# zjuzly/MultiViewStitch

Hardware: AMD Instinct MI355X
Metric: nonrigid_outer_iterations_per_sec (higher is better)
Workload: dtype f64

## Files before the change

multiviewstitch_amd/csrc/deform_handle.cpp:

```cpp
#include "deform_host.h"
#include <chrono>

int check_params(const mvs_deform_params* p) {
    if (!p) { mvs_set_error("params is NULL"); return MVS_E_INVALID_ARG; }
    if (p->top_k < 1 || p->top_k > 8 || p->graph_k < 0 || p->graph_k > 63 || p->smooth_sweeps < 0 ||
        p->arap_iters < 1 || p->arap_iters > 8 || p->cg_max_iters < 1 || !(p->cg_tol > 0)) {
        mvs_set_error("params out of range (top_k 1..8, graph_k 0..63, arap_iters 1..8, cg_tol > 0)");
        return MVS_E_INVALID_ARG;
    }
    return MVS_OK;
}

static void free_nodes(mvs_deform_s* h) {
    if (h->arena_nodes) { (void)hipFree(h->arena_nodes); h->arena_nodes = nullptr; }
    h->d_nodes = nullptr; h->d_nbr = nullptr; h->d_node_pts = nullptr; h->d_node_nrm = nullptr; h->d_ctrl_raw = nullptr;
    h->d_ctrl_a = nullptr; h->d_ctrl_b = nullptr; h->d_valid = nullptr; h->d_d2min = nullptr; h->d_counts = nullptr;
    h->d_records = nullptr; h->d_top_idx = nullptr; h->d_heavy = nullptr; h->d_heavy2 = nullptr;
    h->d_prev_d2 = nullptr; h->d_prev_node = nullptr; h->d_knn_ws = nullptr;
    h->d_near_prev = nullptr; h->d_lim = nullptr; h->d_mid = nullptr; h->d_mid2 = nullptr; h->d_ng_sync = nullptr;
    h->near_age = 0; h->graph_prev_nn = 0;
    h->prev_valid = false;
    h->d_ctrl_final = nullptr; h->K = 0; h->nbr_k = 0; h->h_nodes.clear();
    h->graph_ready_nn = 0; h->weights_ready = false; h->heavy_pending = nullptr;
}
// ... 58 lines not shown
    if (!h) return MVS_OK;
    (void)hipSetDevice(h->device);
    if (h->stream) (void)hipStreamSynchronize(h->stream);
    free_nodes(h);
    for (void* a : {h->arena_mesh, h->arena_tab, h->arena_target, h->arena_probe}) if (a) (void)hipFree(a);
    if (h->d_slots) (void)hipFree(h->d_slots);
    if (h->d_cheb) (void)hipFree(h->d_cheb);
    if (h->d_sh) { (void)hipFree(h->d_sh); h->d_sh = nullptr; }
    if (h->h_ctl) { (void)hipHostFree((void*)h->h_ctl); h->h_ctl = nullptr; }
    if (h->timing.h_sample) { (void)hipHostFree(h->timing.h_sample); h->timing.h_sample = nullptr; }
    for (auto& pr : h->timing.pending) { (void)hipEventDestroy(pr.second.first); (void)hipEventDestroy(pr.second.second); }
    for (hipEvent_t e : h->timing.event_pool) (void)hipEventDestroy(e);
    if (h->own_stream) stream_release(h->device, h->own_stream);
    delete h;
    return MVS_OK;
}

static int install_nodes(mvs_deform_s* h, const int32_t* vertex_idx, int64_t K) {
    free_nodes(h);
    h->K = K;
    h->h_nodes.assign(vertex_idx, vertex_idx + K);
    const size_t ws_bytes = K >= 1024 ? knn_grid_ws_bytes((int)K) : 0;
    auto lay = [&](Arena& a) {
        h->d_heavy = a.take<int32_t>((size_t)K + 1); h->d_heavy2 = a.take<int32_t>((size_t)K + 1);
        h->d_valid = a.take<uint8_t>((size_t)K);
        h->d_nodes = a.take<int32_t>(K); h->d_node_pts = a.take<double>((size_t)K * 3); h->d_node_nrm = a.take<double>((size_t)K * 3);
        h->d_ctrl_raw = a.take<double>((size_t)K * 3); h->d_ctrl_a = a.take<double>((size_t)K * 3); h->d_ctrl_b = a.take<double>((size_t)K * 3);
        h->d_d2min = a.take<float>(K); h->d_counts = a.take<int32_t>((size_t)K * 2);
        h->d_prev_d2 = a.take<float>(K); h->d_prev_node = a.take<double>((size_t)K * 3);
        h->d_near_prev = a.take<double>((size_t)K * 3); h->d_lim = a.take<float>(K);
        h->d_mid = a.take<int32_t>((size_t)K + 1); h->d_mid2 = a.take<int32_t>((size_t)K + 1);
        h->d_ng_sync = a.take<unsigned long long>(32);
        h->d_records = a.take<mvs_cand>((size_t)K * 8); h->d_top_idx = a.take<int64_t>((size_t)K * 8);
        h->d_nbr = a.take<int32_t>((size_t)K * 64);
        h->d_knn_ws = ws_bytes ? (void*)a.take<char>(ws_bytes) : nullptr;
    };
    {
        Arena a; lay(a);
        HIPCHK(hipMalloc(&h->arena_nodes, a.off + 256));
        Arena b; b.base = (char*)h->arena_nodes; lay(b);
    }
    HIPCHK(hipMemsetAsync(h->d_heavy, 0, sizeof(int32_t), h->stream)); HIPCHK(hipMemsetAsync(h->d_heavy2, 0, sizeof(int32_t), h->stream));
    HIPCHK(hipMemsetAsync(h->d_mid, 0, sizeof(int32_t), h->stream)); HIPCHK(hipMemsetAsync(h->d_mid2, 0, sizeof(int32_t), h->stream));
    HIPCHK(hipMemsetAsync(h->d_ng_sync, 0, sizeof(unsigned long long) * 32, h->stream));
    h->ng_pass = 0;
    HIPCHK(hipMemsetAsync(h->d_valid, 0, (size_t)std::max<int64_t>(K, 1), h->stream));
    h->heavy_flip = 0;
    HIPCHK(hipMemsetAsync(h->d_is_ctrl, 0, sizeof(int32_t) * h->V, h->stream));
    if (K) HIPCHK(hipMemcpyAsync(h->d_nodes, h->h_nodes.data(), sizeof(int32_t) * K, hipMemcpyHostToDevice, h->stream));
    launch_gather_nodes(h->d_pts, h->d_nrm, h->d_nodes, (int)K, h->d_node_pts, h->d_node_nrm, h->stream, h->d_is_ctrl);
    if (K) HIPCHK(hipMemcpyAsync(h->d_ctrl_raw, h->d_node_pts, sizeof(double) * K * 3, hipMemcpyDeviceToDevice, h->stream));
    h->d_ctrl_final = h->d_ctrl_raw;
    h->cg_iters = 0;
    for (int i = 0; i < 8; ++i) { h->cg_plan[i] = 0; h->ras_plan[i] = 0; h->bump_seq[i] = 0; h->ras_hist_n[i] = 0; }
    h->ras_mix_any = 0; h->ras_mix_calm = 0; h->assoc_passes = 0;
    HIPCHK(hipMemsetAsync(h->d_ctl, 0, sizeof(double) * 4, h->stream));
    h->ras_a = 0.0; h->ras_m = 0;
    return MVS_OK;
}

int mvs_deform_set_nodes(mvs_deform_t h, const int32_t* vertex_idx, int64_t K) {
    MVS_TRACE();
    if (!h || K < 0 || (K > 0 && !vertex_idx)) { mvs_set_error("bad arguments"); return MVS_E_INVALID_ARG; }
    HIPCHK(hipSetDevice(h->device));
    std::vector<char> seen(h->V, 0);
    for (int64_t k = 0; k < K; ++k) {
        const int v = vertex_idx[k];
        if (v < 0 || v >= h->V) { mvs_set_error("node %lld: vertex index out of range", (long long)k); return MVS_E_INVALID_ARG; }
        if (seen[v]) { mvs_set_error("node %lld: vertex %d listed twice", (long long)k, v); return MVS_E_INVALID_ARG; }
        seen[v] = 1;
    }
    return install_nodes(h, vertex_idx, K);
}

int mvs_deform_set_vertices(mvs_deform_t h, const double* points, const double* normals) {
    MVS_TRACE();
    if (!h || !points) { mvs_set_error("bad arguments"); return MVS_E_INVALID_ARG; }
    HIPCHK(hipSetDevice(h->device));
    HIPCHK(hipStreamSynchronize(h->stream));
    HIPCHK(hipMemcpyAsync(h->d_pts, points, sizeof(double) * 3 * (size_t)h->V, hipMemcpyHostToDevice, h->stream));
    if (normals) HIPCHK(hipMemcpyAsync(h->d_nrm, normals, sizeof(double) * 3 * (size_t)h->V, hipMemcpyHostToDevice, h->stream));
    if (h->K > 0) {
        launch_gather_nodes(h->d_pts, h->d_nrm, h->d_nodes, (int)h->K, h->d_node_pts, h->d_node_nrm, h->stream);
        HIPCHK(hipMemcpyAsync(h->d_ctrl_raw, h->d_node_pts, sizeof(double) * h->K * 3, hipMemcpyDeviceToDevice, h->stream));
        HIPCHK(hipMemsetAsync(h->d_valid, 0, (size_t)h->K, h->stream));
        h->d_ctrl_final = h->d_ctrl_raw;
    }
    h->graph_ready_nn = 0; h->weights_ready = false; h->heavy_pending = nullptr; h->graph_in_local = false;
    h->near_age = 0;
    HIPCHK(hipStreamSynchronize(h->stream));
    return mvs_check_hip(hipGetLastError(), "set_vertices");
}

int mvs_deform_sample_nodes(mvs_deform_t h, int knn, int64_t* K) {
    MVS_TRACE();
    if (!h || knn < 1 || knn > 64) { mvs_set_error("knn must be 1..64"); return MVS_E_INVALID_ARG; }
    HIPCHK(hipSetDevice(h->device));
    const int64_t V = h->V;
    const auto t0 = std::chrono::steady_clock::now();
    auto lap = [&](const char* what) {
        if (mvs_debug_level()) fprintf(stderr, "[mvs] sample_nodes: %s at %.3f ms\n", what, std::chrono::duration<double, std::milli>(std::chrono::steady_clock::now() - t0).count());
    };
    const size_t tab_bytes = (sizeof(int32_t) * (size_t)V * knn + 255) & ~(size_t)255;
    const size_t ws_bytes = V >= 1024 ? knn_grid_ws_bytes((int)V) : 0;
    int32_t* tab = nullptr;
    int rc;
    {
// ... 146 lines not shown
```

multiviewstitch_amd/csrc/deform_iterate.cpp:

```cpp
#include "deform_host.h"

extern "C" {

int mvs_deform_iterate(mvs_deform_t h, const mvs_deform_params* p, int n_outer, mvs_deform_stats* stats) {
    MVS_TRACE();
    int rc = ready(h, p, true);
    if (rc) return rc;
    if (n_outer < 0) return MVS_E_INVALID_ARG;
    int done = 0;
    if (!stats && h->cg_iters > 0) {
        const CgPlan cg = probe_cg(h, *p);
        for (int o = 0; o < n_outer; ++o) {
            enqueue_assoc_local(h, *p);
            rc = enqueue_solve(h, *p, h->d_ctrl_raw, true, cg, true);
            if (rc) return rc;
        }
        return MVS_OK;
    }
    int status = MVS_OK;
    BatchAcc acc;
    acc.st = h->last;
    while (done < n_outer) {
        const bool calibrated = h->cg_iters > 0;
        const int batch = calibrated ? std::min(n_outer - done, MAX_BATCH) : 1;
        CgPlan cg = probe_cg(h, *p);
        for (int o = 0; o < batch; ++o) {
            if (calibrated && o > 0) {
                if ((rc = throttle(h))) return rc;
                peek_ring(h, *p, use_ras(h, *p));
                cg = probe_cg(h, *p);
            }
            enqueue_assoc_local(h, *p);
            rc = enqueue_solve(h, *p, h->d_ctrl_raw, true, cg);
            if (rc) return rc;
        }
        mvs_deform_stats st;
        rc = harvest(h, *p, cg, &st);
        if (rc < 0) return rc;
        if (rc > 0) status = rc;
        acc.add(st);
        done += batch;
    }
    acc.finish(&h->last, done);
    if (stats) *stats = h->last;
    return status;
}

int mvs_deform_assoc_dmin(mvs_deform_t h, const mvs_deform_params* p, float* d2min_dev) {
    MVS_TRACE();
    int rc = ready(h, p, true);
    if (rc) return rc;
    if (!d2min_dev) return MVS_E_INVALID_ARG;
    h->near_age = 0;
    Tic t = tic(h, "assoc");
    launch_assoc_dmin(h->grid, h->d_node_pts, (int)h->K, d2min_dev, h->stream, h->prev_valid ? h->d_prev_d2 : nullptr, h->d_prev_node);
    toc(t, 1);
    return mvs_check_hip(hipGetLastError(), "assoc_dmin");
}
int mvs_deform_assoc_select(mvs_deform_t h, const mvs_deform_params* p, const float* d2min_dev, mvs_cand* records_dev,
                            int32_t* counts_dev) {
    MVS_TRACE();
    int rc = ready(h, p, true);
    if (rc) return rc;
    if (!d2min_dev || !records_dev || !counts_dev) return MVS_E_INVALID_ARG;
// ... 112 lines not shown
```

multiviewstitch_amd/csrc/deform_pass.cpp:

```cpp
#include "deform_host.h"

AssocLists assoc_lists(const mvs_deform_s* h, int flip) {
    if (flip) return {h->d_heavy2, h->d_heavy, h->d_mid2, h->d_mid};
    return {h->d_heavy, h->d_heavy2, h->d_mid, h->d_mid2};
}

void enqueue_assoc_local(mvs_deform_s* h, const mvs_deform_params& p) {
    Tic t = tic(h, "assoc");
    const int K = (int)h->K;
    const AssocLists l = assoc_lists(h, h->heavy_flip);
    int32_t *cur = l.heavy, *nxt = l.heavy_next, *mcur = l.mid, *mnxt = l.mid_next;
    h->heavy_flip ^= 1;
    if (h->near_age >= 2 && h->grid.P > 0 && K > 0 && p.graph_k + 1 <= 16 && MVS_KNOB("MVS_ASSOC_BOUNDED", 1, 0, 1) != 0.0) {
        const int nn = p.graph_k + 1;
        const bool graph_here = h->d_knn_ws != nullptr && knn_grid_is_single(K) && ensure_nbr(h, nn) == MVS_OK;
        const bool bounded_graph = graph_here && h->graph_prev_nn == nn && K >= nn;
        const bool w = graph_here && use_ras(h, p);
        const bool build_in_all = graph_here && assoc_all_builds_grid(K) && MVS_KNOB("MVS_NG_IN_ALL", 1, 0, 1) != 0.0;
        launch_assoc_prep(h->grid, h->d_node_pts, K, h->d_d2min, h->d_near_prev, h->d_lim, cur, mcur, (graph_here && !build_in_all) ? h->d_knn_ws : nullptr, h->stream);
        launch_assoc_all(h->grid, h->d_node_pts, h->d_node_nrm, K, p, h->d_lim, h->d_d2min, h->d_records, h->d_counts, cur, mcur, nxt, mnxt, h->d_ctrl_raw,
                         h->d_valid, h->d_top_idx, nn, h->d_nbr, graph_here ? h->d_knn_ws : nullptr, bounded_graph, w ? &h->sell : nullptr, h->d_pts,
                         arap_grid_blocks(h->sell), h->stream, build_in_all ? h->d_ng_sync : nullptr, build_in_all ? ++h->ng_pass : 0);
        h->assoc_passes++;
        h->near_age++;
// ... 162 lines not shown

void finalize_pass(mvs_deform_s* h, const mvs_deform_params& p, const RasPlan& rp, const RasPass& c, const SolveState& st) {
    hipStream_t s = h->stream;
    const int K = (int)h->K, V = (int)h->V;
    double* host_ctl = const_cast<double*>(h->h_ctl);
    Tic t = tic(h, "finalize");
    int n = 1;
    if (p.update_normals) {
        launch_arap_finalize(h->sell, p.arap_iters, p.arap_tol, h->d_energy, st.x_cur, h->d_pts, h->d_info, nullptr, nullptr, nullptr, p.cg_tol, h->d_ctl, c.slot, host_ctl, st.prev_scal, s, c.nl, c.demand_local, (double)(h->seq_enqueued + 1));
        launch_vertex_normals(h->d_pts, h->d_faces, h->d_vf_ptr, h->d_vf, V, h->d_nrm, s);
        launch_gather_nodes(h->d_pts, h->d_nrm, h->d_nodes, K, h->d_node_pts, h->d_node_nrm, s);
        n = 3;
    } else {
        launch_arap_finalize(h->sell, p.arap_iters, p.arap_tol, h->d_energy, st.x_cur, h->d_pts, h->d_info, h->d_nrm, h->d_node_pts, h->d_node_nrm, p.cg_tol, h->d_ctl, c.slot, host_ctl, st.prev_scal, s, c.nl, c.demand_local, (double)(h->seq_enqueued + 1));
    }
    toc(t, n);
    if (st.sampling) {
        auto& T = h->timing;
        const int ss = ras_slot_size(h);
        const size_t nslots = (size_t)rp.total(p.arap_iters);
        T.sample_off.push_back(T.sample_used);
        (void)hipMemcpy2DAsync(T.h_sample + T.sample_used, 8 * sizeof(double), h->d_ras_slots + 3 * (size_t)h->ras.NPpad, (size_t)ss * sizeof(double),
                               8 * sizeof(double), nslots, hipMemcpyDeviceToHost, s);
        T.sample_used += nslots * 8;
    }
}

}

int enqueue_solve(mvs_deform_s* h, const mvs_deform_params& p, const double* ctrl_src, bool graph_smooth, const CgPlan& plan, bool safe_local) {
    Smoothed sm;
    sm.ctrl = ctrl_src;
    if (graph_smooth) {
        int rc = graph_and_smooth(h, p, &sm);
        if (rc) return rc;
    }
    if (!sm.last_sweep.out) h->d_ctrl_final = const_cast<double*>(sm.ctrl);
    const bool ras = use_ras(h, p);
    if (ras) update_mix_state(h, p.arap_iters);
    const RasPlan rp = probe_ras(h);
    int rc = ras ? ensure_ras_slots(h, p.arap_iters) : ensure_slots(h, p.arap_iters, plan);
    if (rc) return rc;
    weights_and_prepare(h, sm, ras);
    RasPass c;
    c.slot = (int)(h->seq_enqueued % MVS_RING);
    c.fused = ras && ras_can_fuse_local(h);
    c.safe_local = safe_local || h->saw_abandon;
    c.nl = ras ? ras_local_parts(h) : 0;
    c.demand_local = (c.fused && !c.safe_local) ? 1 : 0;
    SolveState st;
    st.x_cur = h->d_sol;
    st.sampling = ras && h->timing.mode == 3 && timed(h, "cg") && sample_room(h, rp.total(p.arap_iters));
    if (st.sampling) h->timing.sample_pass_first.push_back((int)h->timing.samples.size());
    if (ras) ras_solves(h, p, rp, c, st);
    else cg_solves(h, p, plan, c.slot);
    finalize_pass(h, p, rp, c, st);
    h->graph_ready_nn = 0; h->weights_ready = false;
    h->seq_enqueued++;
    return MVS_OK;
}
```

multiviewstitch_amd/csrc/deform_plan.cpp:

```cpp
#include "deform_host.h"
#include <sched.h>

constexpr int RAS_SPARES = 1;
static int ras_spares(int used) { return RAS_SPARES + used / 8; }
#define RAS_A_FLOOR MVS_KNOB("MVS_RAS_FLOOR", 0.01, 0.001, 0.06)
constexpr double PEEK_AT = 1.0;

constexpr int RAS_FIRST_PLANS[8] = {7, 6, 5, 5, 5, 5, 5, 5};
constexpr int RAS_MAX_SWEEPS = 128;
#define RAS_MIX_PLAN ((int)MVS_KNOB("MVS_MIX_PLAN", 11, 2, 128))
constexpr int RAS_MIX_OFF = 7, RAS_MIX_CALM = 16;
void update_mix_state(mvs_deform_s* h, int arap_iters) {
    bool any_long = false, all_short = true;
    for (int it = 0; it < arap_iters; ++it) {
        if (h->ras_plan[it] >= RAS_MIX_PLAN) any_long = true;
        if (h->ras_plan[it] > RAS_MIX_OFF) all_short = false;
    }
    if (any_long) { h->ras_mix_any = 1; h->ras_mix_calm = 0; }
    else if (h->ras_mix_any) {
        if (!all_short) h->ras_mix_calm = 0;
        else if (++h->ras_mix_calm >= RAS_MIX_CALM) { h->ras_mix_any = 0; h->ras_mix_calm = 0; }
    }
}

RasPlan probe_ras(const mvs_deform_s* h) {
    RasPlan r;
    for (int i = 0; i < 8; ++i) r.n[i] = h->ras_plan[i] > 0 ? h->ras_plan[i] : RAS_FIRST_PLANS[i];
    if (h->ras_mix_any) for (int i = 0; i < 8; ++i) r.n[i] = std::max(r.n[i], RAS_MIX_PLAN);
    const int cap = h->dbg.plan_cap > 0 ? h->dbg.plan_cap : (int)MVS_KNOB("MVS_RAS_PLAN_CAP", 0, 0, 128);
    if (cap > 0) for (int i = 0; i < 8; ++i) r.n[i] = std::min(r.n[i], cap);
    return r;
}

int ensure_ras_slots(mvs_deform_s* h, int arap_iters) {
    if ((int64_t)RAS_MAX_SWEEPS * arap_iters > h->ras_slots_cap || !h->d_ras_slots) { mvs_set_error("sweep slots not provisioned"); return MVS_E_STATE; }
    return MVS_OK;
}

int ensure_slots(mvs_deform_s* h, int arap_iters, const CgPlan& cg) {
    int64_t need = cg.total_slots(arap_iters) * MVS_CG_SLOT;
    if (need > h->slots_cap) {
        need += need / 2;
        if (h->d_slots) (void)hipFree(h->d_slots);
        int rc = dmalloc(&h->d_slots, (size_t)need);
        if (rc) return rc;
        h->slots_cap = need;
    }
    return MVS_OK;
}

constexpr int THROTTLE_LAG = 3;

int throttle(mvs_deform_s* h) {
    if (!h->h_ctl) return MVS_OK;
    for (unsigned spins = 0;; ++spins) {
        const uint64_t done = (uint64_t)h->h_ctl[MVS_CTL_SEQ];
        if (h->seq_enqueued <= done + THROTTLE_LAG) return MVS_OK;
        if ((spins & 0x3ff) == 0x3ff) {
            const hipError_t e = hipStreamQuery(h->stream);
            if (e == hipSuccess) return MVS_OK;
            if (e != hipErrorNotReady) return mvs_check_hip(e, "stream (throttle)");
            sched_yield();
        }
    }
}

void peek_ring(mvs_deform_s* h, const mvs_deform_params& p, bool ras) {
    if (!h->h_ctl) return;
    uint64_t done = (uint64_t)h->h_ctl[MVS_CTL_SEQ];
    const uint64_t due = h->seq_enqueued > (uint64_t)THROTTLE_LAG ? h->seq_enqueued - THROTTLE_LAG : 0;
    if (done > due) done = due;
    uint64_t q = h->seq_peeked;
    if (q >= done) return;
    if (done > MVS_RING && q < done - MVS_RING) q = done - MVS_RING;
    const double tol2 = PEEK_AT * PEEK_AT * p.cg_tol * p.cg_tol;
    const bool plan_lowering = MVS_KNOB("MVS_PLAN_LOWER", 1, 0, 1) != 0.0;
    for (; q < done; ++q) {
        const volatile double* row = h->h_ctl + MVS_CTL_RING + (q % MVS_RING) * 8;
        const volatile double* used = h->h_ctl + MVS_CTL_USED + (q % MVS_RING) * 8;
        for (int it = 0; it < p.arap_iters; ++it) {
            const double rel2 = row[it];
            if (rel2 < 0.0) continue;
            int want = 0;
            if (ras) {
                if (h->ras_plan[it] <= 0) continue;
                const int u = (int)used[it];
                if (u != 0) {
                    const int ran = std::abs(u) + (u < 0 ? 1 : 0);
                    want = ran + ras_spares(ran);
                    int* hist = h->ras_hist[it];
                    if (h->ras_hist_n[it] == 4) { hist[0] = hist[1]; hist[1] = hist[2]; hist[2] = hist[3]; hist[3] = ran; }
                    else hist[h->ras_hist_n[it]++] = ran;
                    const int HN = (int)MVS_KNOB("MVS_PLAN_HIST", 4, 1, 4);
                    if (plan_lowering && h->ras_hist_n[it] >= HN && u > 0) {
                        int m = 0;
                        for (int k = h->ras_hist_n[it] - HN; k < h->ras_hist_n[it]; ++k) m = std::max(m, hist[k]);
                        const int low = m + ras_spares(m);
                        if (low < h->ras_plan[it] && want <= low) {
                            if (mvs_debug_level()) fprintf(stderr, "[mvs] pass %llu solve %d: plan %d -> %d (the last four passes ran <= %d sweeps)\n",
                                                                (unsigned long long)q, it, h->ras_plan[it], low, m);
                            h->ras_plan[it] = low;
                        }
                    }
                }
                if (rel2 > tol2) want = std::max(want, h->ras_plan[it] + ras_spares(h->ras_plan[it]) + 1);
                want = std::min(RAS_MAX_SWEEPS, want);
                if (want > h->ras_plan[it]) {
                    if (mvs_debug_level()) fprintf(stderr, "[mvs] pass %llu solve %d ran %d of %d sweeps (ended at %.2e of cg_tol): plan %d from pass %llu on\n",
                                                        (unsigned long long)q, it, std::abs(u), h->ras_plan[it], std::sqrt(rel2) / p.cg_tol, want, (unsigned long long)h->seq_enqueued);
                    h->ras_plan[it] = want;
                }
            } else if (h->cg_plan[it] > 0 && rel2 > tol2 && q >= h->bump_seq[it]) {
                h->cg_plan[it] = std::min(p.cg_max_iters, h->cg_plan[it] + std::max(2, h->cg_plan[it] / 8));
                h->bump_seq[it] = h->seq_enqueued;
            }
        }
    }
    h->seq_peeked = done;
}

namespace {
struct Judgement {
    double worst2 = 0.0, last_worst2 = 0.0; int solves = 0, missed = 0; bool esc = false; double last_row[8];
    int rows = 0; int used[MVS_RING][8];
};
int read_judgement(mvs_deform_s* h, const mvs_deform_params& p, Judgement* j) {
    double ctl[MVS_CTL_SIZE];
    HIPCHK(hipMemcpyAsync(ctl, h->d_ctl, sizeof ctl, hipMemcpyDeviceToHost, h->stream));
    HIPCHK(hipStreamSynchronize(h->stream));
    j->esc = ctl[MVS_CTL_ESC] != 0.0;
    for (int it = 0; it < 8; ++it)
        if (ctl[MVS_CTL_GAVEUP + it] > h->gaveup_seen[it]) {
            h->gaveup_seen[it] = ctl[MVS_CTL_GAVEUP + it];
            h->saw_abandon = true;
        }
    if (mvs_debug_level()) fprintf(stderr, "[mvs] predicted stops: true / predicted residual (running maximum) %.2f\n", std::sqrt(std::max(1.0, ctl[MVS_CTL_PSAFE])));
    j->worst2 = ctl[MVS_CTL_WORST];
    j->missed = (int)ctl[MVS_CTL_MISSED];
    j->solves = (int)ctl[MVS_CTL_SOLVES];
    const double* row = ctl + MVS_CTL_RING + ((h->seq_enqueued + MVS_RING - 1) % MVS_RING) * 8;
    for (int it = 0; it < 8; ++it) { j->last_row[it] = row[it]; if (it < p.arap_iters && row[it] > j->last_worst2) j->last_worst2 = row[it]; }
    {
        const uint64_t since = std::min<uint64_t>(h->seq_enqueued - h->seq_harvested, MVS_RING);
        j->rows = (int)since;
        for (uint64_t q = 0; q < since; ++q) {
            const double* u = ctl + MVS_CTL_USED + ((h->seq_enqueued - 1 - q) % MVS_RING) * 8;
            for (int it = 0; it < 8; ++it) { const int v = (int)u[it]; j->used[q][it] = v < 0 ? 1 - v : v; }
        }
        h->seq_harvested = h->seq_enqueued;
    }
    HIPCHK(hipMemsetAsync(h->d_ctl, 0, sizeof(double) * 4, h->stream));
    h->seq_peeked = h->seq_enqueued;
    return MVS_OK;
}
int judged_status(const Judgement& j, const mvs_deform_params& p) {
    if (j.missed == 0) return MVS_OK;
    mvs_set_error("%d of %d global solves ended above cg_tol = %.1e (worst relative residual %.3e)%s", j.missed, j.solves, p.cg_tol,
                  std::sqrt(j.worst2), j.esc ? "; the device switched the remaining solves to the strong local-solve coefficients" : "");
    return MVS_W_UNCONVERGED;
}

struct PassReadback {
    std::vector<double> ered;
    int32_t info[8];
    std::vector<uint8_t> valid;
    Judgement jd;
    explicit PassReadback(const mvs_deform_s* h) : ered(MVS_ERED_SIZE), valid(h->K) {}
    int run() const { return info[0]; }
    int download(mvs_deform_s* h, const mvs_deform_params& p) {
        HIPCHK(hipMemcpyAsync(ered.data(), h->d_energy, sizeof(double) * MVS_ERED_SIZE, hipMemcpyDeviceToHost, h->stream));
        HIPCHK(hipMemcpyAsync(info, h->d_info, sizeof info, hipMemcpyDeviceToHost, h->stream));
        if (h->K) HIPCHK(hipMemcpyAsync(valid.data(), h->d_valid, (size_t)h->K, hipMemcpyDeviceToHost, h->stream));
        return read_judgement(h, p, &jd);
    }
    mvs_deform_stats fill(mvs_deform_s* h, const mvs_deform_params& p, int cg_iters, int launches, int active, mvs_deform_stats* st) const {
        mvs_deform_stats out{};
        out.arap_iters_run = run();
        out.cg_iters = cg_iters;
        for (int i = 0; i < 8; ++i) out.energy[i] = i < p.arap_iters ? ered[MVS_ERED_FIN + i] : 0.0;
        out.cg_rel_residual = std::sqrt(std::max(0.0, jd.last_worst2));
        out.worst_rel_residual_in_batch = std::sqrt(std::max(0.0, jd.worst2));
        out.solves_in_batch = jd.solves;
        out.unconverged_solves = jd.missed;
        out.escalated = jd.esc ? 1 : 0;
        out.cg_launches = launches; out.cg_active = active;
        int nv = 0;
        for (uint8_t v : valid) nv += v;
        out.n_valid = nv;
        h->last = out;
        if (st) *st = out;
        collect_timers(h);
        return out;
    }
};

}

int harvest(mvs_deform_s* h, const mvs_deform_params& p, const CgPlan& plan, mvs_deform_stats* st) {
    if (use_ras(h, p)) return harvest_ras(h, p, st);
    const size_t n = (size_t)plan.total_slots(p.arap_iters) * MVS_CG_SLOT;
    std::vector<double> slots(n);
    PassReadback rb(h);
// ... 8 lines not shown
    for (int it = 0; it < run; ++it) {
        const double* S = slots.data() + plan.offset(it);
        const int cg = plan.n[it];
        int first = -1;
        auto gamma_of = [&](int i, int c) {
            if (i < cg) return S[(size_t)i * MVS_CG_SLOT + MVS_CG_FIN + 3 + c];
            double g = 0.0;
            for (int b = 0; b < nb; ++b) g += S[(size_t)i * MVS_CG_SLOT + c * MVS_NBMAX + b];
            return g;
        };
        for (int i = 0; i <= cg; ++i) {
            bool frozen = true;
            for (int c = 0; c < 3; ++c) {
                const double gam = gamma_of(i, c), bn = S[MVS_CG_FIN + 6 + c];
                if (gam > 0.0 && gam > STOP_AT * STOP_AT * p.cg_tol * p.cg_tol * bn) frozen = false;
            }
            if (frozen) { first = i; break; }
        }
        if (first < 0) { all_conv = false; h->cg_plan[it] = std::min(p.cg_max_iters, 2 * cg); first = cg; }
        else h->cg_plan[it] = std::min(p.cg_max_iters, first + first / 8 + 2);
        launches += cg; active += first;
        if (mvs_debug_level()) fprintf(stderr, "[mvs] arap it %d: CG frozen at %d of %d (gamma0 %.3e bn %.3e), true residual %.3e\n", it, first, cg, gamma_of(0, 0), S[MVS_CG_FIN + 6], std::sqrt(std::max(0.0, jd.last_row[it])));
    }
    for (int it = run; it < p.arap_iters; ++it)
        if (h->cg_plan[it] == 0 || h->cg_iters == 0) h->cg_plan[it] = h->cg_plan[std::max(0, run - 1)];
    h->cg_iters = 1;
    const int cg = plan.max(p.arap_iters);
    const mvs_deform_stats out = rb.fill(h, p, cg, launches, active, st);
    if (!all_conv && cg >= p.cg_max_iters) {
        mvs_set_error("global solve did not reach cg_tol in cg_max_iters=%d (rel residual %.3e)", cg, out.worst_rel_residual_in_batch);
        return MVS_E_SOLVER;
    }
    return judged_status(jd, p);
}

int harvest_ras(mvs_deform_s* h, const mvs_deform_params& p, mvs_deform_stats* st, const RasPlan* used) {
    const RasPlan rp = used ? *used : probe_ras(h);
    const int ss = ras_slot_size(h), NP = h->ras.NP, NPpad = h->ras.NPpad;
    const size_t nslots = (size_t)rp.total(p.arap_iters);
    std::vector<double> fin(nslots * 8);
    std::vector<int32_t> iters(nslots * NP);
    PassReadback rb(h);
    HIPCHK(hipMemcpy2DAsync(fin.data(), 8 * sizeof(double), h->d_ras_slots + 3 * (size_t)NPpad, (size_t)ss * sizeof(double), 8 * sizeof(double), nslots,
                            hipMemcpyDeviceToHost, h->stream));
    HIPCHK(hipMemcpyAsync(iters.data(), h->d_ras_iters, iters.size() * sizeof(int32_t), hipMemcpyDeviceToHost, h->stream));
    int rc = rb.download(h, p);
    if (rc) return rc;
    const Judgement& jd = rb.jd;
    const int run = rb.run();
    const double tol2 = p.cg_tol * p.cg_tol;
    int launches = 0, active = 0, max_local = 0, worst_first = 0;
    bool all_conv = true;
    size_t slot = 0;
    for (int it = 0; it < p.arap_iters; ++it) {
        const int n = rp.n[it];
        if (it >= run) { slot += n; continue; }
        const double* F = fin.data() + (slot + n - 1) * 8;
        const double bn[3] = {F[3], F[4], F[5]};
        const bool idle = F[6] != 0.0;
        const int ran = (int)F[7];
        const double final2 = jd.last_row[it];
        auto rel2_at = [&](int i) {
            double worst = 0.0;
            for (int c = 0; c < 3; ++c) {
                const double g = fin[(slot + i) * 8 + c];
                if (g > 0.0 && bn[c] > 0.0) worst = std::max(worst, g / bn[c]);
                else if (g > 0.0) worst = INFINITY;
            }
            return worst;
        };
        for (int i = 0; i < n; ++i) {
            int mx = 0;
            for (int q = 0; q < NP; ++q) mx = std::max(mx, iters[(slot + i) * NP + q]);
            max_local += mx;
        }
        launches += n; active += ran;
        const bool ok = final2 >= 0.0 && final2 <= tol2;
        if (!ok) { all_conv = false; h->ras_plan[it] = std::min(RAS_MAX_SWEEPS, 2 * n); worst_first = std::max(worst_first, n); }
        else {
            int most = ran + (idle ? 0 : 1);
            for (int q = 0; q < jd.rows; ++q) most = std::max(most, jd.used[q][it]);
            h->ras_plan[it] = std::min(RAS_MAX_SWEEPS, most + ras_spares(most));
            if (!h->ras_mix_any) worst_first = std::max(worst_first, ran - 1);
        }
        if (mvs_debug_level()) {
            fprintf(stderr, "[mvs] arap it %d: %d of %d planned sweeps ran%s (true final residual %.3e) -> plan %d\n", it, ran, n, idle ? "" : " — no spare left",
                    std::sqrt(std::max(0.0, final2)), h->ras_plan[it]);
            if (mvs_debug_level() >= 2) {
                fprintf(stderr, "[mvs]   residual of each sweep's input:");
                for (int i = 0; i < std::min(n - 1, ran); ++i) fprintf(stderr, " %.2e", std::sqrt(rel2_at(i)));
                fprintf(stderr, "\n");
            }
        }
        slot += n;
    }
    {
        double a0; int m0;
        ras_default_bracket(h, &a0, &m0);
        double a = h->ras_a > 0.0 ? h->ras_a : a0;
        if (!all_conv || jd.esc || worst_first > 9) {
            a = std::max(a / 3.0, RAS_A_FLOOR);
        } else if (worst_first <= 4 && a < a0) {
            a = std::min(a0, a * 1.5);
            for (int it = 0; it < run; ++it) h->ras_plan[it] = std::min(RAS_MAX_SWEEPS, h->ras_plan[it] + 2);
        }
        if (a != h->ras_a) { h->ras_a = a; h->ras_m = ras_steps_for(a); }
        if (mvs_debug_level()) fprintf(stderr, "[mvs] patch solver bracket a = %.4f, %d steps per sweep\n", h->ras_a, h->ras_m);
    }
    for (int it = run; it < p.arap_iters; ++it)
        if (h->ras_plan[it] == 0) h->ras_plan[it] = h->ras_plan[std::max(0, run - 1)];
    rb.fill(h, p, max_local, launches, active, st);
    h->cg_iters = std::max(h->cg_iters, 1);
    return judged_status(jd, p);
}

CgPlan probe_cg(const mvs_deform_s* h, const mvs_deform_params& p) {
    CgPlan c;
    for (int i = 0; i < 8; ++i)
        c.n[i] = (h->cg_iters > 0 && h->cg_plan[i] > 0) ? std::min(h->cg_plan[i], p.cg_max_iters) : std::min(p.cg_max_iters, 192);
    return c;
}
```

multiviewstitch_amd/csrc/engine.h:

```cpp
#ifndef MVS_ENGINE_H_
#define MVS_ENGINE_H_

#include <hip/hip_runtime.h>
#include <stdint.h>
#include <string>
#include <vector>
#include <map>
#include "../../include/mvs.h"

void mvs_set_error(const char* fmt, ...);
int  mvs_check_hip(hipError_t e, const char* what);
#define HIPCHK(x) do { int _rc = mvs_check_hip((x), #x); if (_rc) return _rc; } while (0)

struct GridDev {
    float    minx, miny, minz;
    float    h, inv_h;
    int32_t  nx, ny, nz;
    int64_t  P;
    int64_t  index_base;
    const float4*  spos;
    const double*  tpos;
    const double*  tnrm;
    const int32_t* cell_start;
    int32_t  NX, NY, NZ;
    const int32_t* coarse_start;
};

struct SellDev {
    int32_t  V, nslices;
    int32_t  single_pass;
    const int32_t* slice_off;
    const int32_t* col;
    const int32_t* opp0;
    const int32_t* opp1;
    double*        w;
    double*        diag;
    const int32_t* is_ctrl;
};

struct ChebCoef { double c0, c1[32], c2[32]; };

struct RasDev {
    int32_t NP, NPpad, W, LS;
    const int32_t* pnloc;
    const int32_t* pown;
    const int32_t* l2g;
    const int16_t* lcol;
    const int32_t* gent;
    const int32_t* gcol;
    int32_t HS;
    const int32_t* pnh;
    const int32_t* hl2g;
};

#define MVS_NBMAX 256
#define MVS_CG_FIN (6 * MVS_NBMAX)
#define MVS_CG_SLOT (MVS_CG_FIN + 16)
#define MVS_ERED_IT (7 * MVS_NBMAX)
#define MVS_ERED_FIN (8 * MVS_ERED_IT)
#define MVS_ERED_SIZE (MVS_ERED_FIN + 8)

// ... 64 lines not shown
    int64_t V = 0, F = 0, K = 0, P = 0;
    double *d_pts = nullptr, *d_nrm = nullptr, *d_sol = nullptr, *d_rot = nullptr;
    int32_t *d_faces = nullptr, *d_vf_ptr = nullptr, *d_vf = nullptr;
    SellDev sell{};
    int32_t *d_slice_off = nullptr, *d_col = nullptr, *d_opp0 = nullptr, *d_opp1 = nullptr, *d_is_ctrl = nullptr;
    double *d_w = nullptr, *d_diag = nullptr;
    int64_t n_entries = 0;
    std::vector<int32_t> h_nodes;
    int32_t *d_nodes = nullptr, *d_nbr = nullptr;
    void *d_knn_ws = nullptr;
    int nbr_k = 0;
    double *d_node_pts = nullptr, *d_node_nrm = nullptr, *d_ctrl_raw = nullptr, *d_ctrl_a = nullptr, *d_ctrl_b = nullptr;
    double *d_ctrl_final = nullptr;
    uint8_t *d_valid = nullptr;
    float *d_d2min = nullptr;
    int32_t *d_counts = nullptr;
    mvs_cand *d_records = nullptr;
    int64_t *d_top_idx = nullptr;
    int32_t *d_heavy = nullptr;
    int32_t *d_heavy2 = nullptr;
    double* d_near_prev = nullptr;
    float* d_lim = nullptr;
    int32_t *d_mid = nullptr, *d_mid2 = nullptr;
    int near_age = 0;
    unsigned long long* d_ng_sync = nullptr;
    unsigned long long ng_pass = 0;
    int graph_prev_nn = 0;
    float* d_prev_d2 = nullptr;
    double* d_prev_node = nullptr;
    bool prev_valid = false;
    int graph_ready_nn = 0;
    bool weights_ready = false;
    const int32_t* heavy_pending = nullptr;
    int heavy_flip = 0;
    GridDev grid{};
    float4 *d_spos = nullptr;
    double *d_tpos = nullptr, *d_tnrm = nullptr;
    int32_t *d_cell_start = nullptr, *d_coarse_cnt = nullptr;
    bool has_target = false;
    double *d_rws[2] = {nullptr, nullptr}, *d_p = nullptr, *d_coef = nullptr;
    double *d_slots = nullptr;
    double *d_energy = nullptr;
    int32_t *d_info = nullptr;
    int64_t slots_cap = 0;
    int cg_iters = 0;
    int cg_plan[8] = {0, 0, 0, 0, 0, 0, 0, 0};
    RasDev ras{};
    bool has_ras = false;
    int64_t ras_rows = 0;
    int ras_block = 1024;
    double *d_ras_x2 = nullptr, *d_ras_b = nullptr, *d_ras_slots = nullptr, *d_ras_pw = nullptr, *d_ras_pd = nullptr;
    int32_t *d_ras_iters = nullptr;
    int64_t ras_slots_cap = 0;
    int ras_plan[8] = {0, 0, 0, 0, 0, 0, 0, 0};
    double ras_a = 0.0;
    int ras_m = 0;
    double* d_ctl = nullptr;
    unsigned* d_bar = nullptr;
    void* d_sh = nullptr;
    int64_t sh_K = 0; int sh_nranks = 0; size_t sh_off_pack = 0, sh_off_all = 0;
    size_t sh_off_recin = 0, sh_off_cntin = 0, sh_off_tblk = 0, sh_off_tall = 0;
    double* d_bpure = nullptr;
    double* d_ras_tail = nullptr;
    int assoc_passes = 0;
    int ras_mix_any = 0, ras_mix_calm = 0;
    double* d_ras_mixf = nullptr;
    double* d_ras_mixp = nullptr;
    volatile double* h_ctl = nullptr;
    int ras_hist[8][4] = {};
    int ras_hist_n[8] = {};
    bool graph_in_local = false;
    uint64_t seq_enqueued = 0;
    uint64_t seq_peeked = 0;
    uint64_t seq_harvested = 0;
    uint64_t bump_seq[8] = {0, 0, 0, 0, 0, 0, 0, 0};
    struct Timing {
        int mode = 0;
        std::map<std::string, PhaseTimer> timers;
        std::vector<std::pair<std::string, std::pair<hipEvent_t, hipEvent_t>>> pending;
        std::vector<hipEvent_t> event_pool;
        std::map<std::string, int64_t> pending_launches;
        struct SweepSample { int first, n_a, n_b; };
        std::vector<SweepSample> samples;
        std::vector<size_t> sample_off;
        std::vector<int> sample_pass_first;
        double* h_sample = nullptr;
        size_t sample_cap = 0, sample_used = 0;
    } timing;
    mvs_deform_stats last{};
    void* arena_mesh = nullptr;
    void* arena_tab = nullptr;
    void* arena_nodes = nullptr;
    void* arena_target = nullptr;
    size_t arena_target_bytes = 0;
    void* arena_probe = nullptr;
    size_t arena_probe_bytes = 0;
    bool saw_abandon = false;
    double gaveup_seen[8] = {0, 0, 0, 0, 0, 0, 0, 0};
    struct TestHooks {
        int maxspin = 0;
        int plan_cap = 0;
        int skip_wg = -1;
        int group_leave = 0;
    } dbg;
    int group_batches = 0;
    ChebCoef* d_cheb = nullptr;
    ChebCoef h_cheb[2];
    double cheb_a_dev = -1.0; int cheb_m_dev = 0, cheb_m2_dev = 0;
    int32_t* d_deg = nullptr;
};

int grid_build(mvs_deform_s* h, int64_t P, const double* pts_dev, const double* nrm_dev, int64_t index_base);
int scan_exclusive_i32(const int32_t* in, int64_t n, int32_t* out, hipStream_t s);
void launch_assoc_dmin(const GridDev& g, const double* node_pts, int K, float* d2min, hipStream_t s, const float* prev_d2 = nullptr,
                       const double* prev_node = nullptr);
void launch_assoc_select(const GridDev& g, const double* node_pts, const double* node_nrm, int K, int top_k,
                         float* d2min, mvs_cand* rec, int32_t* counts, int32_t* heavy , int heavy_cap,
                         hipStream_t s, bool defer_heavy = false ,
                         float* prev_d2 = nullptr, double* prev_node = nullptr );
void launch_assoc_local(const GridDev& g, const double* node_pts, const double* node_nrm, int K, const mvs_deform_params& p, float* d2min,
                        mvs_cand* rec, int32_t* counts, int32_t* heavy , int32_t* heavy_next ,
                        int heavy_cap, double* controls, uint8_t* valid, int64_t* top_idx, hipStream_t s, bool defer_heavy = false,
                        int nn = 0, int32_t* nbr = nullptr, void* knn_ws = nullptr , int heavy_rows = 0 );
// ... 139 lines not shown
```

Measured before the change: 2179.

## Factor RAS sweep-plan rule into header and feed unseen ring rows at harvest

Moves the adaptive sweep-plan logic (history, spares, raise/lower, mix state) into a shared header with a per-solve plan struct. At harvest, ring rows the host never peeked are now fed through the same rule, replacing the coarse re-provisioning, so plans keep tracking actual sweep use when batches are not followed. The intent is tighter sweep plans with fewer wasted launches. The risk is that plans lowered too far cause more misses and doubling.

```diff
diff --git a/multiviewstitch_amd/csrc/deform_handle.cpp b/multiviewstitch_amd/csrc/deform_handle.cpp
--- a/multiviewstitch_amd/csrc/deform_handle.cpp
+++ b/multiviewstitch_amd/csrc/deform_handle.cpp
@@ -134,7 +134,7 @@
     if (K) HIPCHK(hipMemcpyAsync(h->d_ctrl_raw, h->d_node_pts, sizeof(double) * K * 3, hipMemcpyDeviceToDevice, h->stream));
     h->d_ctrl_final = h->d_ctrl_raw;
     h->cg_iters = 0;
-    for (int i = 0; i < 8; ++i) { h->cg_plan[i] = 0; h->ras_plan[i] = 0; h->bump_seq[i] = 0; h->ras_hist_n[i] = 0; }
+    for (int i = 0; i < 8; ++i) { h->cg_plan[i] = 0; h->ras_plan[i] = RasSolvePlan{}; h->bump_seq[i] = 0; }
     h->ras_mix_any = 0; h->ras_mix_calm = 0; h->assoc_passes = 0;
     HIPCHK(hipMemsetAsync(h->d_ctl, 0, sizeof(double) * 4, h->stream));
     h->ras_a = 0.0; h->ras_m = 0;
diff --git a/multiviewstitch_amd/csrc/deform_iterate.cpp b/multiviewstitch_amd/csrc/deform_iterate.cpp
--- a/multiviewstitch_amd/csrc/deform_iterate.cpp
+++ b/multiviewstitch_amd/csrc/deform_iterate.cpp
@@ -10,6 +10,7 @@
     int done = 0;
     if (!stats && h->cg_iters > 0) {
         const CgPlan cg = probe_cg(h, *p);
+        if (n_outer > 0) h->ring_unfollowed = true;
         for (int o = 0; o < n_outer; ++o) {
             enqueue_assoc_local(h, *p);
             rc = enqueue_solve(h, *p, h->d_ctrl_raw, true, cg, true);
diff --git a/multiviewstitch_amd/csrc/deform_pass.cpp b/multiviewstitch_amd/csrc/deform_pass.cpp
--- a/multiviewstitch_amd/csrc/deform_pass.cpp
+++ b/multiviewstitch_amd/csrc/deform_pass.cpp
@@ -238,6 +238,7 @@
     st.x_cur = h->d_sol;
     st.sampling = ras && h->timing.mode == 3 && timed(h, "cg") && sample_room(h, rp.total(p.arap_iters));
     if (st.sampling) h->timing.sample_pass_first.push_back((int)h->timing.samples.size());
+    if (ras) for (int it = 0; it < 8; ++it) h->ras_plan_ring[c.slot][it] = rp.n[it];
     if (ras) ras_solves(h, p, rp, c, st);
     else cg_solves(h, p, plan, c.slot);
     finalize_pass(h, p, rp, c, st);
diff --git a/multiviewstitch_amd/csrc/deform_plan.cpp b/multiviewstitch_amd/csrc/deform_plan.cpp
--- a/multiviewstitch_amd/csrc/deform_plan.cpp
+++ b/multiviewstitch_amd/csrc/deform_plan.cpp
@@ -1,32 +1,19 @@
 #include "deform_host.h"
 #include <sched.h>
 
-constexpr int RAS_SPARES = 1;
-static int ras_spares(int used) { return RAS_SPARES + used / 8; }
 #define RAS_A_FLOOR MVS_KNOB("MVS_RAS_FLOOR", 0.01, 0.001, 0.06)
 constexpr double PEEK_AT = 1.0;
 
-constexpr int RAS_FIRST_PLANS[8] = {7, 6, 5, 5, 5, 5, 5, 5};
-constexpr int RAS_MAX_SWEEPS = 128;
+constexpr int RAS_MAX_SWEEPS = RAS_RULE_MAX;
 #define RAS_MIX_PLAN ((int)MVS_KNOB("MVS_MIX_PLAN", 11, 2, 128))
 constexpr int RAS_MIX_OFF = 7, RAS_MIX_CALM = 16;
 void update_mix_state(mvs_deform_s* h, int arap_iters) {
-    bool any_long = false, all_short = true;
-    for (int it = 0; it < arap_iters; ++it) {
-        if (h->ras_plan[it] >= RAS_MIX_PLAN) any_long = true;
-        if (h->ras_plan[it] > RAS_MIX_OFF) all_short = false;
-    }
-    if (any_long) { h->ras_mix_any = 1; h->ras_mix_calm = 0; }
-    else if (h->ras_mix_any) {
-        if (!all_short) h->ras_mix_calm = 0;
-        else if (++h->ras_mix_calm >= RAS_MIX_CALM) { h->ras_mix_any = 0; h->ras_mix_calm = 0; }
-    }
+    ras_rule_mix(h->ras_plan, arap_iters, RasMixRule{RAS_MIX_PLAN, RAS_MIX_OFF, RAS_MIX_CALM}, &h->ras_mix_any, &h->ras_mix_calm);
 }
 
 RasPlan probe_ras(const mvs_deform_s* h) {
     RasPlan r;
-    for (int i = 0; i < 8; ++i) r.n[i] = h->ras_plan[i] > 0 ? h->ras_plan[i] : RAS_FIRST_PLANS[i];
-    if (h->ras_mix_any) for (int i = 0; i < 8; ++i) r.n[i] = std::max(r.n[i], RAS_MIX_PLAN);
+    for (int i = 0; i < 8; ++i) r.n[i] = ras_rule_launches(h->ras_plan[i], i, h->ras_mix_any, RAS_MIX_PLAN);
     const int cap = h->dbg.plan_cap > 0 ? h->dbg.plan_cap : (int)MVS_KNOB("MVS_RAS_PLAN_CAP", 0, 0, 128);
     if (cap > 0) for (int i = 0; i < 8; ++i) r.n[i] = std::min(r.n[i], cap);
     return r;
@@ -49,7 +36,28 @@
     return MVS_OK;
 }
 
-constexpr int THROTTLE_LAG = 3;
+#define THROTTLE_LAG ((int)MVS_KNOB("MVS_THROTTLE_LAG", RAS_RULE.lag, 1, 8))
+#define PLAN_HIST ((int)MVS_KNOB("MVS_PLAN_HIST", RAS_RULE.hist, 1, 4))
+
+static void trace_pass(const mvs_deform_s* h, uint64_t q, const int* used, int arap_iters) {
+    if (!mvs_debug_level()) return;
+    fprintf(stderr, "[mvs] pass %llu used", (unsigned long long)q);
+    for (int it = 0; it < arap_iters; ++it) fprintf(stderr, " %d", used[it]);
+    fprintf(stderr, " plan");
+    for (int it = 0; it < arap_iters; ++it) fprintf(stderr, " %d", h->ras_plan_ring[q % MVS_RING][it]);
+    fprintf(stderr, "\n");
+}
+static void feed_rule(mvs_deform_s* h, const mvs_deform_params& p, uint64_t q, int it, int u, double rel2, bool plan_lowering) {
+    const bool missed = rel2 > PEEK_AT * PEEK_AT * p.cg_tol * p.cg_tol;
+    int was = 0;
+    const int what = ras_rule_row(&h->ras_plan[it], u, missed, plan_lowering ? PLAN_HIST : 0, &was);
+    if (!mvs_debug_level() || what == RAS_RULE_KEPT) return;
+    if (what == RAS_RULE_LOWERED)
+        fprintf(stderr, "[mvs] pass %llu solve %d: plan %d -> %d (the last passes ran fewer sweeps)\n", (unsigned long long)q, it, was, h->ras_plan[it].n);
+    else
+        fprintf(stderr, "[mvs] pass %llu solve %d ran %d of %d sweeps (ended at %.2e of cg_tol): plan %d from pass %llu on\n",
+                (unsigned long long)q, it, std::abs(u), was, std::sqrt(rel2) / p.cg_tol, h->ras_plan[it].n, (unsigned long long)h->seq_enqueued);
+}
 
 int throttle(mvs_deform_s* h) {
     if (!h->h_ctl) return MVS_OK;
@@ -78,39 +86,12 @@
     for (; q < done; ++q) {
         const volatile double* row = h->h_ctl + MVS_CTL_RING + (q % MVS_RING) * 8;
         const volatile double* used = h->h_ctl + MVS_CTL_USED + (q % MVS_RING) * 8;
+        if (ras) { int u8[8]; for (int it = 0; it < 8; ++it) u8[it] = (int)used[it]; trace_pass(h, q, u8, p.arap_iters); }
         for (int it = 0; it < p.arap_iters; ++it) {
             const double rel2 = row[it];
             if (rel2 < 0.0) continue;
-            int want = 0;
-            if (ras) {
-                if (h->ras_plan[it] <= 0) continue;
-                const int u = (int)used[it];
-                if (u != 0) {
-                    const int ran = std::abs(u) + (u < 0 ? 1 : 0);
-                    want = ran + ras_spares(ran);
-                    int* hist = h->ras_hist[it];
-                    if (h->ras_hist_n[it] == 4) { hist[0] = hist[1]; hist[1] = hist[2]; hist[2] = hist[3]; hist[3] = ran; }
-                    else hist[h->ras_hist_n[it]++] = ran;
-                    const int HN = (int)MVS_KNOB("MVS_PLAN_HIST", 4, 1, 4);
-                    if (plan_lowering && h->ras_hist_n[it] >= HN && u > 0) {
-                        int m = 0;
-                        for (int k = h->ras_hist_n[it] - HN; k < h->ras_hist_n[it]; ++k) m = std::max(m, hist[k]);
-                        const int low = m + ras_spares(m);
-                        if (low < h->ras_plan[it] && want <= low) {
-                            if (mvs_debug_level()) fprintf(stderr, "[mvs] pass %llu solve %d: plan %d -> %d (the last four passes ran <= %d sweeps)\n",
-                                                                (unsigned long long)q, it, h->ras_plan[it], low, m);
-                            h->ras_plan[it] = low;
-                        }
-                    }
-                }
-                if (rel2 > tol2) want = std::max(want, h->ras_plan[it] + ras_spares(h->ras_plan[it]) + 1);
-                want = std::min(RAS_MAX_SWEEPS, want);
-                if (want > h->ras_plan[it]) {
-                    if (mvs_debug_level()) fprintf(stderr, "[mvs] pass %llu solve %d ran %d of %d sweeps (ended at %.2e of cg_tol): plan %d from pass %llu on\n",
-                                                        (unsigned long long)q, it, std::abs(u), h->ras_plan[it], std::sqrt(rel2) / p.cg_tol, want, (unsigned long long)h->seq_enqueued);
-                    h->ras_plan[it] = want;
-                }
-            } else if (h->cg_plan[it] > 0 && rel2 > tol2 && q >= h->bump_seq[it]) {
+            if (ras) feed_rule(h, p, q, it, (int)used[it], rel2, plan_lowering);
+            else if (h->cg_plan[it] > 0 && rel2 > tol2 && q >= h->bump_seq[it]) {
                 h->cg_plan[it] = std::min(p.cg_max_iters, h->cg_plan[it] + std::max(2, h->cg_plan[it] / 8));
                 h->bump_seq[it] = h->seq_enqueued;
             }
@@ -123,6 +104,8 @@
 struct Judgement {
     double worst2 = 0.0, last_worst2 = 0.0; int solves = 0, missed = 0; bool esc = false; double last_row[8];
     int rows = 0; int used[MVS_RING][8];
+    int unseen = 0; uint64_t unseen_first = 0; int unseen_used[MVS_RING][8]; double unseen_rel2[MVS_RING][8];
+    bool followed = false;
 };
 int read_judgement(mvs_deform_s* h, const mvs_deform_params& p, Judgement* j) {
     double ctl[MVS_CTL_SIZE];
@@ -148,6 +131,15 @@
             for (int it = 0; it < 8; ++it) { const int v = (int)u[it]; j->used[q][it] = v < 0 ? 1 - v : v; }
         }
         h->seq_harvested = h->seq_enqueued;
+        const uint64_t unseen = h->seq_enqueued - h->seq_peeked;
+        j->followed = h->h_ctl && !h->ring_unfollowed && unseen <= MVS_RING;
+        j->unseen = (int)std::min<uint64_t>(unseen, MVS_RING);
+        j->unseen_first = h->seq_enqueued - (uint64_t)j->unseen;
+        for (int k = 0; k < j->unseen; ++k) {
+            const size_t slot = (size_t)((j->unseen_first + k) % MVS_RING) * 8;
+            for (int it = 0; it < 8; ++it) { j->unseen_used[k][it] = (int)ctl[MVS_CTL_USED + slot + it]; j->unseen_rel2[k][it] = ctl[MVS_CTL_RING + slot + it]; }
+        }
+        h->ring_unfollowed = false;
     }
     HIPCHK(hipMemsetAsync(h->d_ctl, 0, sizeof(double) * 4, h->stream));
     h->seq_peeked = h->seq_enqueued;
@@ -262,6 +254,16 @@
     int launches = 0, active = 0, max_local = 0, worst_first = 0;
     bool all_conv = true;
     size_t slot = 0;
+    if (!used) for (int k = 0; k < jd.unseen; ++k) trace_pass(h, jd.unseen_first + k, jd.unseen_used[k], p.arap_iters);
+    const bool follow = jd.followed && !used && !h->ras_mix_any;
+    const bool plan_lowering = MVS_KNOB("MVS_PLAN_LOWER", 1, 0, 1) != 0.0;
+    bool fed[8] = {};
+    for (int it = 0; it < p.arap_iters; ++it) {
+        fed[it] = follow && h->ras_plan[it].n > 0;
+        if (!fed[it]) continue;
+        for (int k = 0; k < jd.unseen; ++k)
+            if (jd.unseen_rel2[k][it] >= 0.0) feed_rule(h, p, jd.unseen_first + k, it, jd.unseen_used[k][it], jd.unseen_rel2[k][it], plan_lowering);
+    }
     for (int it = 0; it < p.arap_iters; ++it) {
         const int n = rp.n[it];
         if (it >= run) { slot += n; continue; }
@@ -286,16 +288,16 @@
         }
         launches += n; active += ran;
         const bool ok = final2 >= 0.0 && final2 <= tol2;
-        if (!ok) { all_conv = false; h->ras_plan[it] = std::min(RAS_MAX_SWEEPS, 2 * n); worst_first = std::max(worst_first, n); }
+        if (!ok) { all_conv = false; ras_rule_miss(&h->ras_plan[it], n); worst_first = std::max(worst_first, n); }
         else {
             int most = ran + (idle ? 0 : 1);
             for (int q = 0; q < jd.rows; ++q) most = std::max(most, jd.used[q][it]);
-            h->ras_plan[it] = std::min(RAS_MAX_SWEEPS, most + ras_spares(most));
+            if (!fed[it]) ras_rule_provision(&h->ras_plan[it], most);
             if (!h->ras_mix_any) worst_first = std::max(worst_first, ran - 1);
         }
         if (mvs_debug_level()) {
             fprintf(stderr, "[mvs] arap it %d: %d of %d planned sweeps ran%s (true final residual %.3e) -> plan %d\n", it, ran, n, idle ? "" : " — no spare left",
-                    std::sqrt(std::max(0.0, final2)), h->ras_plan[it]);
+                    std::sqrt(std::max(0.0, final2)), h->ras_plan[it].n);
             if (mvs_debug_level() >= 2) {
                 fprintf(stderr, "[mvs]   residual of each sweep's input:");
                 for (int i = 0; i < std::min(n - 1, ran); ++i) fprintf(stderr, " %.2e", std::sqrt(rel2_at(i)));
@@ -312,13 +314,13 @@
             a = std::max(a / 3.0, RAS_A_FLOOR);
         } else if (worst_first <= 4 && a < a0) {
             a = std::min(a0, a * 1.5);
-            for (int it = 0; it < run; ++it) h->ras_plan[it] = std::min(RAS_MAX_SWEEPS, h->ras_plan[it] + 2);
+            for (int it = 0; it < run; ++it) ras_rule_weaker_local(&h->ras_plan[it]);
         }
         if (a != h->ras_a) { h->ras_a = a; h->ras_m = ras_steps_for(a); }
         if (mvs_debug_level()) fprintf(stderr, "[mvs] patch solver bracket a = %.4f, %d steps per sweep\n", h->ras_a, h->ras_m);
     }
     for (int it = run; it < p.arap_iters; ++it)
-        if (h->ras_plan[it] == 0) h->ras_plan[it] = h->ras_plan[std::max(0, run - 1)];
+        if (h->ras_plan[it].n == 0) h->ras_plan[it].n = h->ras_plan[std::max(0, run - 1)].n;
     rb.fill(h, p, max_local, launches, active, st);
     h->cg_iters = std::max(h->cg_iters, 1);
     return judged_status(jd, p);
diff --git a/multiviewstitch_amd/csrc/engine.h b/multiviewstitch_amd/csrc/engine.h
--- a/multiviewstitch_amd/csrc/engine.h
+++ b/multiviewstitch_amd/csrc/engine.h
@@ -7,6 +7,7 @@
 #include <vector>
 #include <map>
 #include "../../include/mvs.h"
+#include "ras_plan_rule.h"
 
 void mvs_set_error(const char* fmt, ...);
 int  mvs_check_hip(hipError_t e, const char* what);
@@ -177,7 +178,7 @@
     double *d_ras_x2 = nullptr, *d_ras_b = nullptr, *d_ras_slots = nullptr, *d_ras_pw = nullptr, *d_ras_pd = nullptr;
     int32_t *d_ras_iters = nullptr;
     int64_t ras_slots_cap = 0;
-    int ras_plan[8] = {0, 0, 0, 0, 0, 0, 0, 0};
+    RasSolvePlan ras_plan[8];
     double ras_a = 0.0;
     int ras_m = 0;
     double* d_ctl = nullptr;
@@ -192,8 +193,8 @@
     double* d_ras_mixf = nullptr;
     double* d_ras_mixp = nullptr;
     volatile double* h_ctl = nullptr;
-    int ras_hist[8][4] = {};
-    int ras_hist_n[8] = {};
+    int ras_plan_ring[MVS_RING][8] = {};
+    bool ring_unfollowed = false;
     bool graph_in_local = false;
     uint64_t seq_enqueued = 0;
     uint64_t seq_peeked = 0;
diff --git a/multiviewstitch_amd/csrc/ras_plan_rule.h b/multiviewstitch_amd/csrc/ras_plan_rule.h
--- /dev/null
+++ b/multiviewstitch_amd/csrc/ras_plan_rule.h
@@ -0,0 +1,73 @@
+#ifndef MVS_RAS_PLAN_RULE_H_
+#define MVS_RAS_PLAN_RULE_H_
+
+constexpr int RAS_RULE_MAX = 128;
+constexpr int RAS_RULE_HIST = 4;
+
+struct RasRule { int lag, hist; };
+constexpr RasRule RAS_RULE = {3, 4};
+
+constexpr int RAS_RULE_FIRST[8] = {7, 6, 5, 5, 5, 5, 5, 5};
+
+struct RasSolvePlan {
+    int n = 0;
+    int hist[RAS_RULE_HIST] = {};
+    int hist_n = 0;
+};
+
+inline int ras_rule_spares(int ran) { return 1 + ran / 8; }
+inline int ras_rule_ran(int u) { return u < 0 ? 1 - u : u; }
+inline int ras_rule_cap(int n) { return n < RAS_RULE_MAX ? n : RAS_RULE_MAX; }
+
+enum { RAS_RULE_KEPT = 0, RAS_RULE_RAISED = 1, RAS_RULE_LOWERED = 2 };
+
+inline int ras_rule_row(RasSolvePlan* s, int u, bool missed, int hist_len, int* was = nullptr) {
+    if (was) *was = s->n;
+    if (s->n <= 0) return RAS_RULE_KEPT;
+    int want = 0, what = RAS_RULE_KEPT;
+    if (u != 0) {
+        const int ran = ras_rule_ran(u);
+        want = ran + ras_rule_spares(ran);
+        if (s->hist_n == RAS_RULE_HIST) { for (int k = 1; k < RAS_RULE_HIST; ++k) s->hist[k - 1] = s->hist[k]; s->hist[RAS_RULE_HIST - 1] = ran; }
+        else s->hist[s->hist_n++] = ran;
+        const int want_rows = hist_len > RAS_RULE_HIST ? RAS_RULE_HIST : hist_len;
+        const int hn = want_rows < s->hist_n ? want_rows : s->hist_n;
+        if (hn >= 1 && u > 0) {
+            int m = 0;
+            for (int k = s->hist_n - hn; k < s->hist_n; ++k) m = s->hist[k] > m ? s->hist[k] : m;
+            const int low = m + ras_rule_spares(m);
+            if (low < s->n && want <= low) { s->n = low; what = RAS_RULE_LOWERED; }
+        }
+    }
+    if (missed) { const int more = s->n + ras_rule_spares(s->n) + 1; want = more > want ? more : want; }
+    want = ras_rule_cap(want);
+    if (want > s->n) { s->n = want; what = RAS_RULE_RAISED; }
+    return what;
+}
+
+inline void ras_rule_provision(RasSolvePlan* s, int most) { s->n = ras_rule_cap(most + ras_rule_spares(most)); }
+inline void ras_rule_miss(RasSolvePlan* s, int planned) { s->n = ras_rule_cap(2 * planned); }
+inline void ras_rule_weaker_local(RasSolvePlan* s) { s->n = ras_rule_cap(s->n + 2); }
+
+struct RasMixRule { int mix_plan, off, calm; };
+inline void ras_rule_mix(const RasSolvePlan* s, int solves, const RasMixRule& r, int* any, int* calm) {
+    bool any_long = false, all_short = true;
+    for (int it = 0; it < solves; ++it) {
+        if (s[it].n >= r.mix_plan) any_long = true;
+        if (s[it].n > r.off) all_short = false;
+    }
+    if (any_long) { *any = 1; *calm = 0; }
+    else if (*any) {
+        if (!all_short) *calm = 0;
+        else if (++*calm >= r.calm) { *any = 0; *calm = 0; }
+    }
+}
+inline int ras_rule_launches(const RasSolvePlan& s, int it, int mix_any, int mix_plan) {
+    const int n = s.n > 0 ? s.n : RAS_RULE_FIRST[it];
+    return mix_any && n < mix_plan ? mix_plan : n;
+}
+
+inline int ras_rule_idle(int n, int need) { return n > need + 1 ? n - need - 1 : 0; }
+inline int ras_rule_tail(int n, int need) { return need >= n ? need - n + 1 : 0; }
+
+#endif
```

Result: no change. 2175 (median of 2 runs) (-0.2%).
